# akuhara/RF_INV

Measured on NVIDIA B200. Metric: forward+likelihood evals/sec, higher is better.
Workload: dtype f64

## Files before the change

### rf_inv_b200/build.py

```python
from __future__ import annotations

import os
import shutil
import subprocess
import sys

HERE = os.path.dirname(os.path.abspath(__file__))
CSRC = os.path.join(HERE, "csrc")
SO = os.path.join(HERE, "librfinv_b200.so")
SOURCES = ["capi.cu", "forward.cu", "forward_general.cu", "likelihood.cu", "pt.cu", "comm.cu", "checkpoint.cu", "fp64_peak.cu", "host_io.cu"]
HEADERS = ["rfinv_common.cuh", "rfinv_handle.h", "rfinv_pt.h", os.path.join("..", "..", "include", "rfinv_b200.h")]
NVCC_FLAGS = [
    "-gencode", "arch=compute_100a,code=sm_100a", "-lineinfo", "-O3", "-std=c++17",
    "-Xcompiler", "-fPIC", "-Xcompiler", "-O3", "--expt-relaxed-constexpr", "-Xptxas", "-v",
]


def nvcc_path() -> str:
    for cand in (os.environ.get("NVCC"), shutil.which("nvcc"), "/usr/local/cuda/bin/nvcc"):
        if cand and os.path.exists(cand):
            return cand
    raise RuntimeError("nvcc not found")


def needs_build() -> bool:
    if not os.path.exists(SO):
        return True
    t = os.path.getmtime(SO)
    deps = [os.path.join(CSRC, s) for s in SOURCES + HEADERS] + [os.path.abspath(__file__)]
    return any(os.path.exists(d) and os.path.getmtime(d) > t for d in deps)


def build(force: bool = False, verbose: bool = False) -> str:
    if not force and not needs_build():
        return SO
    objdir = os.path.join(HERE, "build")
    os.makedirs(objdir, exist_ok=True)
    nvcc = nvcc_path()
    objs = []
    procs = []
    env = dict(os.environ)
    host_cxx = "/usr/bin/g++" if os.path.exists("/usr/bin/g++") else "g++"
    for s in SOURCES:
        o = os.path.join(objdir, s.replace(".cu", ".o"))
# ... 23 lines not shown
```

### rf_inv_b200/csrc/capi.cu

```cuda
#include <cstdarg>
#include <cstdio>
#include <cstdlib>
#include <cstring>
#include <cmath>
#include <vector>
#include <algorithm>
#include "rfinv_handle.h"

static thread_local char g_err[1024] = "";

int rfinv_pdl_mode() {
  static const int mode = getenv("RFINV_PDL") ? atoi(getenv("RFINV_PDL")) : 2;
  return mode;
}

int rfinv_arith_switches() {
  auto on = [](const char* name) { return getenv(name) && atoi(getenv(name)) != 0; };
  static const int bits = (on("RFINV_FULL_BAND") ? 1 : 0) | (on("RFINV_QF_DENSE") ? 2 : 0) | (on("RFINV_QF_NOSPLIT") ? 4 : 0);
  return bits;
}

void rfinv_set_error(const char* fmt, ...) {
  va_list ap;
  va_start(ap, fmt);
  vsnprintf(g_err, sizeof(g_err), fmt, ap);
  va_end(ap);
}

namespace {

void build_filter(const rfinv_config& c, std::vector<double>& flt) {
  const int nh = c.nfft / 2 + 1;
  flt.resize((size_t)c.ntrc * nh);
  const double df = 1.0 / (c.delta * c.nfft);
  for (int t = 0; t < c.ntrc; ++t) {
    const double fac_norm = c.nfft * c.a_gus[t] * c.delta / std::sqrt(RFINV_PI);
    for (int i = 0; i < nh; ++i) {
      const double omega = i * 2.0 * RFINV_PI * df;
      const double q = omega / (2.0 * c.a_gus[t]);
      flt[(size_t)t * nh + i] = std::exp(-(q * q)) / fac_norm;
// ... 369 lines not shown
  d.prior_mode = cfg->prior_mode; d.nref = cfg->nref;
  d.ray_common = 1;
  for (int t = 1; t < T; ++t)
    if (cfg->rayps[t] != cfg->rayps[0] || cfg->ipha[t] != cfg->ipha[0]) d.ray_common = 0;
  d.nsmp_pad = ((S + 63) / 64) * 64;
  d.delta = cfg->delta; d.t_start = cfg->t_start; d.sdep = cfg->sdep; d.bdep = cfg->bdep; d.z_ref_min = cfg->z_ref_min; d.dz_ref = cfg->dz_ref;
  d.z_min = cfg->z_min; d.z_max = cfg->z_max; d.h_min = cfg->h_min;
  d.vp_min = cfg->vp_min; d.vp_max = cfg->vp_max; d.vs_min = cfg->vs_min; d.vs_max = cfg->vs_max;
  d.vpvs_min = cfg->vpvs_min; d.vpvs_max = cfg->vpvs_max;
  d.domg = 2.0 * RFINV_PI / (cfg->nfft * cfg->delta);
  for (int t = 0; t < T; ++t) { d.rayp[t] = cfg->rayps[t]; d.ipha[t] = cfg->ipha[t]; }

  std::vector<double> flt;
  build_filter(*cfg, flt);
  band_limits(d, flt);
  std::vector<double2> tw;
  build_twiddles(d.fft_len, tw);
  std::vector<double2> chirp, chirp_b;
  std::vector<double2> twq;
  if (d.fft_general) {
    build_chirp(cfg->nfft, d.fft_len, chirp, chirp_b);
    for (int N = d.fft_len; N > 8; N >>= 3) {
      const int stride = N >> 3, tmul = d.fft_len / N;
      for (int i = 0; i < 7 * stride; ++i) { const int q = i / stride + 1, o = i - (q - 1) * stride; twq.push_back(tw[(size_t)q * o * tmul]); }
    }
  }
  const int Sp = d.nsmp_pad;
  std::vector<double> rpad((size_t)T * Sp * Sp, 0.0);
  for (int t = 0; t < T; ++t)
    for (int i = 0; i < S; ++i)
      for (int j = 0; j < S; ++j)
        rpad[((size_t)t * Sp + i) * Sp + j] =
            0.5 * (h->h_r_inv[((size_t)t * S + i) * S + j] + h->h_r_inv[((size_t)t * S + j) * S + i]);
  std::vector<double> wfac;
  {
    const bool force_dense = (rfinv_arith_switches() & 2) != 0;
    const bool no_split = (rfinv_arith_switches() & 4) != 0;
    const int ntile_dense = Sp / 64;
    std::vector<std::vector<double>> Wt(T);
    std::vector<int> wrows_t(T, 0);
    std::vector<double> a, w, v, a2, w2, v2;
    d.qf_tiles_max = 0;
    int wrows = 64;
    const double rs2 = 0.70710678118654752440;
    for (int t = 0; t < T; ++t) {
      d.qf_rank[t] = 0; d.qf_rank_s[t] = 0; d.qf_split[t] = 0;
      d.qf_tiles[t] = ntile_dense;
      const double* Rm = &rpad[(size_t)t * Sp * Sp];
      auto R = [&](int i, int j) { return Rm[(size_t)i * Sp + j]; };
      int same = -1;
      for (int u = 0; u < t && same < 0; ++u)
        if (std::memcmp(&rpad[(size_t)u * Sp * Sp], Rm, sizeof(double) * (size_t)Sp * Sp) == 0) same = u;
      if (force_dense) {  }
      else if (same >= 0) {
        d.qf_rank[t] = d.qf_rank[same]; d.qf_rank_s[t] = d.qf_rank_s[same]; d.qf_split[t] = d.qf_split[same];
        d.qf_tiles[t] = d.qf_tiles[same]; Wt[t] = Wt[same]; wrows_t[t] = wrows_t[same];
      } else {
        double rmax = 0.0, asym = 0.0;
        for (int i = 0; i < S; ++i)
          for (int j = 0; j < S; ++j) {
            rmax = std::max(rmax, std::fabs(R(i, j)));
            asym = std::max(asym, std::fabs(R(i, j) - R(S - 1 - i, S - 1 - j)));
          }
        const int ha = S / 2, hs = S - ha;
        const bool split = !no_split && rmax > 0.0 && asym <= 1e-10 * rmax && hs <= Sp / 2;
        const double units_dense = 0.5 * ntile_dense * (ntile_dense + 1);
        auto tile_units = [&](int r) { return r / 64 + (r % 64 ? 0.4 : 0.0); };
// ... 62 lines not shown
            for (int e = 0; e < S; ++e) if (w[e] > tol) order.push_back(e);
            std::sort(order.begin(), order.end(), [&](int x, int y) { return w[x] > w[y] || (w[x] == w[y] && x < y); });
            for (int row = 0; row < r; ++row) {
              const int e = order[row];
              const double sc = std::sqrt(w[e]);
              for (int i = 0; i < S; ++i) Wt[t][(size_t)row * Sp + i] = sc * v[(size_t)i * S + e];
            }
          }
        }
      }
      d.qf_tiles_max = std::max(d.qf_tiles_max, d.qf_tiles[t]);
      wrows = std::max(wrows, wrows_t[t]);
    }
    d.qf_wrows = wrows;
    wfac.assign((size_t)T * wrows * Sp, 0.0);
    for (int t = 0; t < T; ++t)
      if (!Wt[t].empty()) std::memcpy(&wfac[(size_t)t * wrows * Sp], Wt[t].data(), sizeof(double) * Wt[t].size());
    {
      int tr = 0;
      for (int t = 0; t < T; ++t) if (d.qf_tiles[t] > d.qf_tiles[tr]) tr = t;
      std::vector<std::pair<double, int>> cost;
      for (int jt = 0; jt < d.qf_tiles_max && jt < RFINV_MAX_QF_TILES; ++jt) {
        double cst;
        if (d.qf_rank[tr] == 0) cst = jt + 1;
        else if (d.qf_split[tr]) {
          const int rs = d.qf_rank_s[tr], ts = (rs + 63) / 64;
          cst = std::min(64, jt < ts ? rs - 64 * jt : (d.qf_rank[tr] - rs) - 64 * (jt - ts));
        } else cst = std::min(64, d.qf_rank[tr] - 64 * jt);
        cost.push_back({-cst, jt});
      }
      std::sort(cost.begin(), cost.end());
      for (size_t q = 0; q < cost.size(); ++q) d.qf_order[q] = cost[q].second;
    }
  }
#define RFINV_TRY(x) do { st = (x); if (st != RFINV_OK) { rfinv_destroy(h); return st; } } while (0)
  RFINV_TRY(upload(flt, &h->d_flt));
  RFINV_TRY(upload(tw, &h->d_tw));
  if (d.fft_general) { RFINV_TRY(upload(chirp, &h->d_chirp)); RFINV_TRY(upload(chirp_b, &h->d_chirp_b)); RFINV_TRY(upload(twq, &h->d_twq)); }
  RFINV_TRY(upload(h->h_obs, &h->d_obs));
  RFINV_TRY(upload(h->h_vp_ref, &h->d_vp_ref));
  RFINV_TRY(upload(h->h_vs_ref, &h->d_vs_ref));
  RFINV_TRY(upload(rpad, &h->d_r_inv));
  RFINV_TRY(upload(wfac, &h->d_w_fac));
#undef RFINV_TRY
  d.flt = h->d_flt; d.tw = h->d_tw; d.chirp = h->d_chirp; d.chirp_b = h->d_chirp_b; d.twq = h->d_twq; d.obs = h->d_obs; d.vp_ref = h->d_vp_ref; d.vs_ref = h->d_vs_ref; d.r_inv = h->d_r_inv; d.w_fac = h->d_w_fac;
  cudaError_t e = cudaStreamCreateWithFlags(&h->stream, cudaStreamNonBlocking);
  if (e != cudaSuccess) { rfinv_set_error("cudaStreamCreate: %s", cudaGetErrorString(e)); rfinv_destroy(h); return RFINV_ERR_CUDA; }
  h->own_stream = true;
  *out = h;
  return RFINV_OK;
}

void rfinv_destroy(rfinv_handle* h) {
  if (!h) return;
  cudaSetDevice(h->device);
  if (h->stream) cudaStreamSynchronize(h->stream);
  h->free_pt();
  rfinv_comm_destroy(h);
  h->free_workspace();
  cudaFree(h->d_flt); cudaFree(h->d_tw); cudaFree(h->d_chirp); cudaFree(h->d_chirp_b); cudaFree(h->d_twq); cudaFree(h->d_obs); cudaFree(h->d_vp_ref); cudaFree(h->d_vs_ref); cudaFree(h->d_r_inv); cudaFree(h->d_w_fac);
  if (h->own_stream && h->stream) cudaStreamDestroy(h->stream);
  if (h->stream_copy) {
    cudaStreamSynchronize(h->stream_copy);
    cudaStreamDestroy(h->stream_copy);
    for (cudaEvent_t e : h->ev_copy) if (e) cudaEventDestroy(e);
  }
  for (int i = 0; i < RFINV_ASYNC_SLOTS; ++i) {
    if (h->async_stream[i]) { cudaStreamSynchronize(h->async_stream[i]); cudaStreamDestroy(h->async_stream[i]); }
    if (h->async_ws[i]) { h->async_ws[i]->release(); delete h->async_ws[i]; }
  }
  for (int i = 0; i < 4; ++i)
    if (h->ev[i]) cudaEventDestroy(h->ev[i]);
  delete h;
}

int32_t rfinv_set_stream(rfinv_handle* h, uint64_t cuda_stream) {
  if (!h) { rfinv_set_error("handle is NULL"); return RFINV_ERR_ARG; }
  if (h->own_stream && h->stream) { cudaStreamSynchronize(h->stream); cudaStreamDestroy(h->stream); }
  h->stream = reinterpret_cast<cudaStream_t>(cuda_stream);
  h->own_stream = false;
  return RFINV_OK;
}

int32_t rfinv_synchronize(rfinv_handle* h) {
  if (!h) { rfinv_set_error("handle is NULL"); return RFINV_ERR_ARG; }
  RFINV_CUDA_CHECK(cudaStreamSynchronize(h->stream));
  return RFINV_OK;
}

int32_t rfinv_last_launch_count(rfinv_handle* h) { return h ? h->launches : 0; }

int32_t rfinv_set_timing(rfinv_handle* h, int32_t enable) {
  if (!h) { rfinv_set_error("handle is NULL"); return RFINV_ERR_ARG; }
// ... 325 lines not shown
```

### rf_inv_b200/csrc/likelihood.cu

```cuda
#include "rfinv_common.cuh"

namespace {

constexpr int TM = 64;
constexpr int TN = 64;
constexpr int TK = 16;
constexpr int LDS_STRIDE = TK + 4;
constexpr int QF_THREADS = 128;
constexpr int QF_CHUNK = 384;

__device__ __forceinline__ void cp_async16(void* smem_dst, const void* gmem_src) {
  const unsigned d = (unsigned)__cvta_generic_to_shared(smem_dst);
  asm volatile("cp.async.cg.shared.global [%0], [%1], 16;\n" ::"r"(d), "l"(gmem_src));
}
__device__ __forceinline__ void cp_async_commit() { asm volatile("cp.async.commit_group;\n" ::); }
template <int N>
__device__ __forceinline__ void cp_async_wait() { asm volatile("cp.async.wait_group %0;\n" ::"n"(N)); }

__device__ __forceinline__ void dmma884(double& c0, double& c1, double a, double b) {
  asm volatile("mma.sync.aligned.m8n8k4.row.col.f64.f64.f64.f64 {%0,%1}, {%2}, {%3}, {%0,%1};\n"
               : "+d"(c0), "+d"(c1) : "d"(a), "d"(b));
}

__global__ void __launch_bounds__(QF_THREADS, 4) quadform_kernel(const DevConfig cfg, int C, const double* __restrict__ misfit,
                                                              double* __restrict__ phi, double* __restrict__ partial,
                                                              int* __restrict__ arrivals, int* __restrict__ work,
                                                              const int* __restrict__ active, int n_active,
                                                              const int* __restrict__ n_active_dev, const double* __restrict__ sig,
                                                              double* __restrict__ logl) {
  __shared__ __align__(16) double sA[2][TM * LDS_STRIDE];
  __shared__ __align__(16) double sB[2][TN * LDS_STRIDE];
  __shared__ int s_rows[TM];
  __shared__ double s_part[2][TM];
  __shared__ int s_next, s_last;
  const int Sp = cfg.nsmp_pad, T = cfg.ntrc;
  const int tid = threadIdx.x, lane = tid & 31, warp = tid >> 5;
  const int wm = warp >> 1, wn = warp & 1;
  const int n_rb_grid = ((active ? n_active : C) + TM - 1) / TM;
  const int ntile = cfg.qf_tiles_max;
  const int n_items = ntile * T * n_rb_grid;
  const int fr = lane >> 2, fk = lane & 3;
  if (tid == 0) s_next = (int)gridDim.x + atomicAdd(work, 1);
  pdl_wait();
  const int n_rows = active ? (n_active_dev ? *n_active_dev : n_active) : C;
  int item = blockIdx.x;
  while (item < n_items) {
    const int nblk = T * n_rb_grid;
    const int chunk = item / (ntile * QF_CHUNK), local = item - chunk * (ntile * QF_CHUNK);
    const int cb = min(QF_CHUNK, nblk - chunk * QF_CHUNK);
    const int jt = cfg.qf_order[local / cb];
    const int blk = chunk * QF_CHUNK + local % cb;
    const int t = blk / n_rb_grid, rb = blk - t * n_rb_grid;
    const int row0 = rb * TM;
    const int rank = cfg.qf_rank[t];
    const int ntile_t = cfg.qf_tiles[t];
    __syncthreads();
    const int next = s_next;
    int next_raw = 0;
    if (tid == 0) next_raw = atomicAdd(work, 1);
    if (row0 < n_rows && jt < ntile_t) {
      if (tid < TM) {
        int r = row0 + tid;
        r = r < n_rows ? r : n_rows - 1;
        s_rows[tid] = active ? active[r] : r;
      }
      __syncthreads();
      const double* __restrict__ Mt = misfit + (size_t)t * C * Sp;
      const double* __restrict__ Rt = rank > 0 ? cfg.w_fac + (size_t)t * cfg.qf_wrows * Sp : cfg.r_inv + (size_t)t * Sp * Sp;
      int jw = 4, koff = 0, nk = (jt + 1) * (TN / TK);
      if (rank > 0) {
        int cols_tile = rank - jt * TN;
        nk = Sp / TK;
        if (cfg.qf_split[t]) {
          const int rs = cfg.qf_rank_s[t], ts = (rs + TN - 1) / TN;
          cols_tile = jt < ts ? rs - jt * TN : (rank - rs) - (jt - ts) * TN;
          koff = jt < ts ? 0 : Sp >> 1;
          nk = (Sp >> 1) / TK;
        }
        const int nfrag = cols_tile >= TN ? 8 : (cols_tile <= 0 ? 0 : (cols_tile + 7) >> 3);
        jw = (nfrag + 1 - wn) >> 1;
      }
      const double* a_src[4];
      int cp_off[4], cp_row[4];
#pragma unroll
      for (int q = 0; q < 4; ++q) {
        const int id = tid + q * QF_THREADS;
        const int row = id >> 3, seg = id & 7;
        cp_row[q] = row;
        cp_off[q] = row * LDS_STRIDE + seg * 2;
        a_src[q] = Mt + (size_t)s_rows[row] * Sp + seg * 2 + koff;
      }
      double acc[4][4][2];
#pragma unroll
      for (int i = 0; i < 4; ++i)
#pragma unroll
        for (int j = 0; j < 4; ++j) acc[i][j][0] = acc[i][j][1] = 0.0;
      const double* b_base = Rt + (size_t)(jt * TN) * Sp + koff;
#pragma unroll
      for (int q = 0; q < 4; ++q) {
        cp_async16(&sA[0][cp_off[q]], a_src[q]);
        cp_async16(&sB[0][cp_off[q]], b_base + (size_t)cp_row[q] * Sp + (cp_off[q] - cp_row[q] * LDS_STRIDE));
      }
      cp_async_commit();
      for (int ks = 0; ks < nk; ++ks) {
        const int cur = ks & 1;
        cp_async_wait<0>();
        __syncthreads();
        if (ks + 1 < nk) {
          const int k0 = (ks + 1) * TK;
#pragma unroll
          for (int q = 0; q < 4; ++q) {
            cp_async16(&sA[cur ^ 1][cp_off[q]], a_src[q] + k0);
            cp_async16(&sB[cur ^ 1][cp_off[q]], b_base + (size_t)cp_row[q] * Sp + k0 + (cp_off[q] - cp_row[q] * LDS_STRIDE));
          }
          cp_async_commit();
        }
        if (rank == 0 && ks == jt * (TN / TK) && jt > 0) {
#pragma unroll
          for (int i = 0; i < 4; ++i)
#pragma unroll
            for (int j = 0; j < 4; ++j) { acc[i][j][0] *= 2.0; acc[i][j][1] *= 2.0; }
        }
        const double* A = &sA[cur][(wm * 32 + fr) * LDS_STRIDE + fk];
        const double* B = &sB[cur][(wn * 8 + fr) * LDS_STRIDE + fk];
#pragma unroll
        for (int kk = 0; kk < TK; kk += 4) {
          double a[4], b[4];
#pragma unroll
          for (int i = 0; i < 4; ++i) a[i] = A[i * 8 * LDS_STRIDE + kk];
#pragma unroll
          for (int j = 0; j < 4; ++j) b[j] = B[j * 16 * LDS_STRIDE + kk];
          if (jw == 4) {
#pragma unroll
            for (int i = 0; i < 4; ++i)
#pragma unroll
              for (int j = 0; j < 4; ++j) dmma884(acc[i][j][0], acc[i][j][1], a[i], b[j]);
          } else {
#pragma unroll
            for (int j = 0; j < 4; ++j)
              if (j < jw) {
#pragma unroll
                for (int i = 0; i < 4; ++i) dmma884(acc[i][j][0], acc[i][j][1], a[i], b[j]);
              }
          }
        }
      }
#pragma unroll
      for (int i = 0; i < 4; ++i) {
        const double* mrow = Mt + (size_t)s_rows[wm * 32 + 8 * i + fr] * Sp + jt * TN + wn * 8 + 2 * fk;
        double v = 0.0;
        if (rank > 0) {
#pragma unroll
          for (int j = 0; j < 4; ++j) { v = fma(acc[i][j][0], acc[i][j][0], v); v = fma(acc[i][j][1], acc[i][j][1], v); }
        } else {
#pragma unroll
          for (int j = 0; j < 4; ++j) {
            const double2 m = *reinterpret_cast<const double2*>(mrow + 16 * j);
            v = fma(acc[i][j][0], m.x, v);
            v = fma(acc[i][j][1], m.y, v);
          }
        }
        v += __shfl_xor_sync(0xffffffffu, v, 1);
        v += __shfl_xor_sync(0xffffffffu, v, 2);
        if (fk == 0) s_part[wn][wm * 32 + 8 * i + fr] = v;
      }
      __syncthreads();
      double* part_t = partial + (size_t)t * C;
      const size_t jstride = (size_t)T * C;
      if (tid < TM && row0 + tid < n_rows) part_t[(size_t)jt * jstride + s_rows[tid]] = s_part[0][tid] + s_part[1][tid];
      __threadfence();
      __syncthreads();
      if (tid == 0) s_last = (atomicAdd(&arrivals[t * n_rb_grid + rb], 1) == ntile_t - 1);
      __syncthreads();
      if (s_last) {
        __threadfence();
        if (tid < TM && row0 + tid < n_rows) {
          const int c = s_rows[tid];
          double v = 0.0;
          for (int j = 0; j < ntile_t; ++j) v += __ldcg(part_t + (size_t)j * jstride + c);
          phi[(size_t)t * C + c] = v;
        }
        if (tid == 0) arrivals[t * n_rb_grid + rb] = 0;
        if (logl) {
          __threadfence();
          __syncthreads();
          if (tid == 0) s_last = (atomicAdd(&arrivals[T * n_rb_grid + rb], 1) == T - 1);
          __syncthreads();
          if (s_last) {
            __threadfence();
            if (tid < TM && row0 + tid < n_rows) {
              const int c = s_rows[tid];
              double ll = 0.0;
              for (int tt = 0; tt < T; ++tt) {
                const double sg = sig[(size_t)tt * C + c];
                const double ph = __ldcg(phi + (size_t)tt * C + c);
                ll = __dsub_rn(__dsub_rn(ll, __ddiv_rn(__dmul_rn(0.5, ph), __dmul_rn(sg, sg))), __dmul_rn((double)cfg.nsmp, log(sg)));
              }
              logl[c] = ll;
            }
            if (tid == 0) arrivals[T * n_rb_grid + rb] = 0;
          }
        }
      }
    } else {
      __syncthreads();
    }
    if (tid == 0) s_next = (int)gridDim.x + next_raw;
    item = next;
  }
  if (tid == 0) {
    __threadfence();
    if (atomicAdd(work + 1, 1) == (int)gridDim.x - 1) { work[0] = 0; work[1] = 0; }
  }
}

__global__ void loglik_kernel(const DevConfig cfg, int C, const double* __restrict__ phi, const double* __restrict__ sig,
                              double* __restrict__ logl) {
  const int c = blockIdx.x * blockDim.x + threadIdx.x;
  if (c >= C) return;
  double ll = 0.0;
  for (int t = 0; t < cfg.ntrc; ++t) {
    const double s = sig[(size_t)t * C + c];
    const double ph = phi[(size_t)t * C + c];
    ll = __dsub_rn(__dsub_rn(ll, __ddiv_rn(__dmul_rn(0.5, ph), __dmul_rn(s, s))), __dmul_rn((double)cfg.nsmp, log(s)));
  }
  logl[c] = ll;
}

}

size_t rfinv_quadform_partial_doubles(const DevConfig& cfg, int C) { return (size_t)(cfg.nsmp_pad / TN + 1) * cfg.ntrc * C; }
size_t rfinv_quadform_counter_ints(const DevConfig& cfg, int C) { return (size_t)((C + TM - 1) / TM) * (cfg.ntrc + 1) + 4; }

int rfinv_launch_quadform(const DevConfig& cfg, int C, const double* misfit, double* phi, double* partial, int* counters,
                          const int* active, int n_active, const int* n_active_dev, cudaStream_t stream, const double* sig,
                          double* logl) {
  const int n_rows = active ? n_active : C;
  if (n_rows == 0) return RFINV_OK;
  const size_t ntile = cfg.qf_tiles_max;
  int* work = counters;
  int* arrivals = counters + 4;
  static int resident_of_device[64] = {0};
  int dev = 0;
  RFINV_CUDA_CHECK(cudaGetDevice(&dev));
  long long resident = (dev >= 0 && dev < 64) ? resident_of_device[dev] : 0;
  if (resident == 0) {
    int per_sm = 0, n_sm = 0;
    RFINV_CUDA_CHECK(cudaDeviceGetAttribute(&n_sm, cudaDevAttrMultiProcessorCount, dev));
    RFINV_CUDA_CHECK(cudaOccupancyMaxActiveBlocksPerMultiprocessor(&per_sm, quadform_kernel, QF_THREADS, 0));
    resident = (long long)n_sm * (per_sm < 1 ? 1 : per_sm);
    if (dev >= 0 && dev < 64) resident_of_device[dev] = (int)resident;
  }
  const long long items = (long long)ntile * cfg.ntrc * ((n_rows + TM - 1) / TM);
  RFINV_CUDA_CHECK(rfinv_launch_pdl(2, quadform_kernel, dim3((unsigned)(items < resident ? items : resident)), dim3(QF_THREADS), 0, stream, cfg, C,
                                    misfit, phi, partial, arrivals, work, active, n_active, n_active_dev, sig, logl));
  return RFINV_OK;
}

int rfinv_launch_loglik(const DevConfig& cfg, int C, const double* phi, const double* sig, double* logl,
                        cudaStream_t stream) {
  if (C == 0) return RFINV_OK;
  loglik_kernel<<<(C + 255) / 256, 256, 0, stream>>>(cfg, C, phi, sig, logl);
  RFINV_CUDA_CHECK(cudaGetLastError());
  return RFINV_OK;
}
```

### rf_inv_b200/csrc/rfinv_common.cuh

```cuda
#pragma once
#include <cuda_runtime.h>
#include <stdint.h>
#include <math.h>
#include <map>
#include <mutex>
#include <utility>
#include "../../include/rfinv_b200.h"

#define RFINV_MAX_TRC 16
#define RFINV_MAX_K 64
#define RFINV_MAX_LAY (RFINV_MAX_K + 2)
#define RFINV_MAX_QF_TILES 64

#define RFINV_PI 3.1415926535897931

struct DevConfig {
  int ntrc, nfft, nh, nsmp;
  int log2n;
  int fft_general, nfft_p2, fft_len;
  int deconv_mode, vp_mode, k_min, k_max, prior_mode, nref, ray_common;
  int nsmp_pad;
  double bdep;
  double delta, t_start, sdep, z_ref_min, dz_ref, z_min, z_max, h_min;
  double vp_min, vp_max, vs_min, vs_max, vpvs_min, vpvs_max;
  double domg;
  double rayp[RFINV_MAX_TRC];
  int ipha[RFINV_MAX_TRC];
  int jbins[RFINV_MAX_TRC];
  int jb_max;
  const double* flt;
  const double2* tw;
  const double2* twq;
  const double2* chirp;
  const double2* chirp_b;
  const double* obs;
  const double* vp_ref;
  const double* vs_ref;
  const double* r_inv;
  const double* w_fac;
  int qf_rank[RFINV_MAX_TRC];
  int qf_split[RFINV_MAX_TRC];
  int qf_rank_s[RFINV_MAX_TRC];
  int qf_tiles[RFINV_MAX_TRC];
  int qf_tiles_max, qf_wrows;
  int qf_order[RFINV_MAX_QF_TILES];
};

struct ModelBatch {
  int C;
  const int* k;
  const double* z;
  const double* dvp;
  const double* dvs;
  const double* sig;
  const int* active;
  int n_active;
  const int* n_active_dev;
  int chain_major = 0;
};

__host__ __device__ __forceinline__ int f_nint(double x) {
  return x >= 0.0 ? (int)floor(x + 0.5) : -(int)floor(-x + 0.5);
}

__device__ __forceinline__ double vp_to_rho(double a1) {
  double a2 = __dmul_rn(a1, a1), a3 = __dmul_rn(a2, a1), a4 = __dmul_rn(a3, a1), a5 = __dmul_rn(a4, a1);
  double p = __dmul_rn((double)1.6612f, a1);
  p = __dsub_rn(p, __dmul_rn((double)0.4721f, a2));
  p = __dadd_rn(p, __dmul_rn((double)0.0671f, a3));
  p = __dsub_rn(p, __dmul_rn((double)0.0043f, a4));
  p = __dadd_rn(p, __dmul_rn((double)0.000106f, a5));
  return p;
}

__device__ __forceinline__ bool layer_velocity(const DevConfig& cfg, double zc, double d_vs, double d_vp, double& alpha,
                                               double& beta) {
  int iz = f_nint(__ddiv_rn(__dsub_rn(zc, cfg.z_ref_min), cfg.dz_ref)) + 1;
  iz = iz < 1 ? 1 : (iz > cfg.nref ? cfg.nref : iz);
// ... 75 lines not shown
```

### rf_inv_b200/csrc/rfinv_handle.h

```cpp
#pragma once
#include <vector>
#include "rfinv_common.cuh"

struct PtState;

struct EvalWorkspace {
  int cap = 0;
  int* d_k = nullptr;
  double *d_z = nullptr, *d_dvp = nullptr, *d_dvs = nullptr, *d_sig = nullptr, *d_stage = nullptr;
  double *d_misfit = nullptr, *d_phi = nullptr, *d_logl = nullptr, *d_rft_full = nullptr, *d_scratch = nullptr;
  uint8_t* d_valid = nullptr;
  double* d_qpart = nullptr;
  int* d_qcnt = nullptr;
  size_t cap_rft_full = 0;
  int grow(const DevConfig& dc, const rfinv_config& cfg, int device, int C);
  void release();
};

constexpr int RFINV_ASYNC_SLOTS = 2;
constexpr int RFINV_UPLOAD_PIECES = 4;

struct rfinv_handle : EvalWorkspace {
  int device = 0;
  cudaStream_t stream = nullptr;
  bool own_stream = false;
  rfinv_config cfg;
  std::vector<double> h_rayps, h_a_gus, h_obs, h_vp_ref, h_vs_ref, h_sig_min, h_sig_max, h_r_inv;
  std::vector<int32_t> h_ipha;
  DevConfig dc;
  double* d_flt = nullptr;
  double2* d_tw = nullptr;
  double2 *d_chirp = nullptr, *d_chirp_b = nullptr, *d_twq = nullptr;
  double* d_obs = nullptr;
  double* d_vp_ref = nullptr;
  double* d_vs_ref = nullptr;
  double* d_r_inv = nullptr;
  double* d_w_fac = nullptr;
  cudaStream_t stream_copy = nullptr;
  cudaEvent_t ev_copy[RFINV_UPLOAD_PIECES + 2] = {};
  EvalWorkspace* async_ws[RFINV_ASYNC_SLOTS] = {};
  cudaStream_t async_stream[RFINV_ASYNC_SLOTS] = {};
  bool async_pending[RFINV_ASYNC_SLOTS] = {};
  int launches = 0;
  bool timing = false;
  cudaEvent_t ev[4] = {nullptr, nullptr, nullptr, nullptr};
  PtState* pt = nullptr;
  void* comm = nullptr;
  int comm_world = 1, comm_rank = 0;

  int ensure_capacity(int C) { if (C > cap) invalidate_pt_graphs(); return grow(dc, cfg, device, C); }
  void invalidate_pt_graphs();
  void free_workspace() { release(); }
  void free_pt();
  int eval_device(int C, const int* k, const double* z, const double* dvp, const double* dvs, const double* sig,
                  double* logl, double* rft_smp, double* rft_full, uint8_t* is_valid, const int* active, int n_active,
                  const ModelBatch* layout = nullptr, EvalWorkspace* w = nullptr, cudaStream_t s = nullptr,
                  bool prep_done = false,
                  cudaEvent_t before_quadform = nullptr);
};

int rfinv_comm_allgather(rfinv_handle* h, const double* send, double* recv, size_t count, cudaStream_t s);
extern "C" int32_t rfinv_comm_destroy(rfinv_handle* h);
int rfinv_comm_peer_setup(rfinv_handle* h);
void rfinv_comm_peer_release(rfinv_handle* h);
int rfinv_pt_fix_assigned_bins(rfinv_handle* h);
int rfinv_pt_reserve_lhist(rfinv_handle* h, int upto);
int rfinv_arith_switches();
```

Baseline: 12.93 million.

## Compute factored quadratic form with int8 tcgen05 MMA via fp64 digit-plane emulation

After: 12.04 million (median of 6 runs). 6.9% lower.

```diff
diff --git a/rf_inv_b200/build.py b/rf_inv_b200/build.py
--- a/rf_inv_b200/build.py
+++ b/rf_inv_b200/build.py
@@ -9,7 +9,7 @@
 CSRC = os.path.join(HERE, "csrc")
 SO = os.path.join(HERE, "librfinv_b200.so")
 SOURCES = ["capi.cu", "forward.cu", "forward_general.cu", "likelihood.cu", "pt.cu", "comm.cu", "checkpoint.cu", "fp64_peak.cu", "host_io.cu"]
-HEADERS = ["rfinv_common.cuh", "rfinv_handle.h", "rfinv_pt.h", os.path.join("..", "..", "include", "rfinv_b200.h")]
+HEADERS = ["rfinv_common.cuh", "qf_int8.cuh", "rfinv_handle.h", "rfinv_pt.h", os.path.join("..", "..", "include", "rfinv_b200.h")]
 NVCC_FLAGS = [
     "-gencode", "arch=compute_100a,code=sm_100a", "-lineinfo", "-O3", "-std=c++17",
     "-Xcompiler", "-fPIC", "-Xcompiler", "-O3", "--expt-relaxed-constexpr", "-Xptxas", "-v",
diff --git a/rf_inv_b200/csrc/capi.cu b/rf_inv_b200/csrc/capi.cu
--- a/rf_inv_b200/csrc/capi.cu
+++ b/rf_inv_b200/csrc/capi.cu
@@ -6,6 +6,7 @@
 #include <vector>
 #include <algorithm>
 #include "rfinv_handle.h"
+#include "qf_int8.cuh"
 
 static thread_local char g_err[1024] = "";
 
@@ -441,7 +442,8 @@
       for (int j = 0; j < S; ++j)
         rpad[((size_t)t * Sp + i) * Sp + j] =
             0.5 * (h->h_r_inv[((size_t)t * S + i) * S + j] + h->h_r_inv[((size_t)t * S + j) * S + i]);
-  std::vector<double> wfac;
+  std::vector<double> wfac, wqs;
+  std::vector<int8_t> wq;
   {
     const bool force_dense = (rfinv_arith_switches() & 2) != 0;
     const bool no_split = (rfinv_arith_switches() & 4) != 0;
@@ -570,6 +572,33 @@
       std::sort(cost.begin(), cost.end());
       for (size_t q = 0; q < cost.size(); ++q) d.qf_order[q] = cost[q].second;
     }
+    const int nsl = Sp / QI_SW;
+    const size_t slab_bytes = (size_t)QI_PLANES * QI_TN * QI_SW, tile_bytes = nsl * slab_bytes;
+    wq.assign((size_t)T * d.qf_tiles_max * tile_bytes, 0);
+    wqs.assign((size_t)T * wrows, 0.0);
+    for (int t = 0; t < T; ++t) {
+      if (d.qf_rank[t] == 0) continue;
+      const int K = d.qf_split[t] ? Sp / 2 : Sp, ts = d.qf_split[t] ? (d.qf_rank_s[t] + 63) / 64 : d.qf_tiles[t];
+      if (K > QI_KMAX || K % QI_SW) { rfinv_set_error("quadratic form: K = %d outside the exact int8 range", K); rfinv_destroy(h); return RFINV_ERR_ARG; }
+      for (int jt = 0; jt < d.qf_tiles[t]; ++jt) {
+        const int koff = jt < ts ? 0 : Sp / 2;
+        int8_t* tile = &wq[((size_t)t * d.qf_tiles_max + jt) * tile_bytes];
+        for (int n = 0; n < QI_TN; ++n) {
+          const double* col = &wfac[((size_t)t * wrows + 64 * jt + n) * Sp + koff];
+          uint32_t mx = 0;
+          for (int k = 0; k < K; ++k) { uint64_t b; std::memcpy(&b, &col[k], 8); mx = std::max(mx, (uint32_t)(b >> 32) & 0x7fffffffu); }
+          const int E = qi_exp(mx);
+          const double sc = qi_scale_in(E);
+          wqs[(size_t)t * wrows + 64 * jt + n] = qi_scale_out(E);
+          for (int k = 0; k < K; ++k) {
+            uint32_t lo, hi;
+            qi_digits(col[k] * sc, lo, hi);
+            int8_t* slab = tile + (size_t)(k / QI_SW) * slab_bytes + qi_sw_offset(n, (k % QI_SW) >> 4) + (k & 15);
+            for (int p = 0; p < QI_PLANES; ++p) slab[(size_t)p * QI_TN * QI_SW] = qi_plane_byte(lo, hi, p);
+          }
+        }
+      }
+    }
   }
 #define RFINV_TRY(x) do { st = (x); if (st != RFINV_OK) { rfinv_destroy(h); return st; } } while (0)
   RFINV_TRY(upload(flt, &h->d_flt));
@@ -579,9 +608,10 @@
   RFINV_TRY(upload(h->h_vp_ref, &h->d_vp_ref));
   RFINV_TRY(upload(h->h_vs_ref, &h->d_vs_ref));
   RFINV_TRY(upload(rpad, &h->d_r_inv));
-  RFINV_TRY(upload(wfac, &h->d_w_fac));
+  RFINV_TRY(upload(wq, &h->d_w_q));
+  RFINV_TRY(upload(wqs, &h->d_w_qscale));
 #undef RFINV_TRY
-  d.flt = h->d_flt; d.tw = h->d_tw; d.chirp = h->d_chirp; d.chirp_b = h->d_chirp_b; d.twq = h->d_twq; d.obs = h->d_obs; d.vp_ref = h->d_vp_ref; d.vs_ref = h->d_vs_ref; d.r_inv = h->d_r_inv; d.w_fac = h->d_w_fac;
+  d.flt = h->d_flt; d.tw = h->d_tw; d.chirp = h->d_chirp; d.chirp_b = h->d_chirp_b; d.twq = h->d_twq; d.obs = h->d_obs; d.vp_ref = h->d_vp_ref; d.vs_ref = h->d_vs_ref; d.r_inv = h->d_r_inv; d.w_q = h->d_w_q; d.w_qscale = h->d_w_qscale;
   cudaError_t e = cudaStreamCreateWithFlags(&h->stream, cudaStreamNonBlocking);
   if (e != cudaSuccess) { rfinv_set_error("cudaStreamCreate: %s", cudaGetErrorString(e)); rfinv_destroy(h); return RFINV_ERR_CUDA; }
   h->own_stream = true;
@@ -596,7 +626,7 @@
   h->free_pt();
   rfinv_comm_destroy(h);
   h->free_workspace();
-  cudaFree(h->d_flt); cudaFree(h->d_tw); cudaFree(h->d_chirp); cudaFree(h->d_chirp_b); cudaFree(h->d_twq); cudaFree(h->d_obs); cudaFree(h->d_vp_ref); cudaFree(h->d_vs_ref); cudaFree(h->d_r_inv); cudaFree(h->d_w_fac);
+  cudaFree(h->d_flt); cudaFree(h->d_tw); cudaFree(h->d_chirp); cudaFree(h->d_chirp_b); cudaFree(h->d_twq); cudaFree(h->d_obs); cudaFree(h->d_vp_ref); cudaFree(h->d_vs_ref); cudaFree(h->d_r_inv); cudaFree(h->d_w_q); cudaFree(h->d_w_qscale);
   if (h->own_stream && h->stream) cudaStreamDestroy(h->stream);
   if (h->stream_copy) {
     cudaStreamSynchronize(h->stream_copy);
diff --git a/rf_inv_b200/csrc/likelihood.cu b/rf_inv_b200/csrc/likelihood.cu
--- a/rf_inv_b200/csrc/likelihood.cu
+++ b/rf_inv_b200/csrc/likelihood.cu
@@ -1,4 +1,5 @@
 #include "rfinv_common.cuh"
+#include "qf_int8.cuh"
 
 namespace {
 
@@ -52,8 +53,7 @@
     const int blk = chunk * QF_CHUNK + local % cb;
     const int t = blk / n_rb_grid, rb = blk - t * n_rb_grid;
     const int row0 = rb * TM;
-    const int rank = cfg.qf_rank[t];
-    const int ntile_t = cfg.qf_tiles[t];
+    const int ntile_t = cfg.qf_rank[t] == 0 ? cfg.qf_tiles[t] : 0;
     __syncthreads();
     const int next = s_next;
     int next_raw = 0;
@@ -66,20 +66,8 @@
       }
       __syncthreads();
       const double* __restrict__ Mt = misfit + (size_t)t * C * Sp;
-      const double* __restrict__ Rt = rank > 0 ? cfg.w_fac + (size_t)t * cfg.qf_wrows * Sp : cfg.r_inv + (size_t)t * Sp * Sp;
-      int jw = 4, koff = 0, nk = (jt + 1) * (TN / TK);
-      if (rank > 0) {
-        int cols_tile = rank - jt * TN;
-        nk = Sp / TK;
-        if (cfg.qf_split[t]) {
-          const int rs = cfg.qf_rank_s[t], ts = (rs + TN - 1) / TN;
-          cols_tile = jt < ts ? rs - jt * TN : (rank - rs) - (jt - ts) * TN;
-          koff = jt < ts ? 0 : Sp >> 1;
-          nk = (Sp >> 1) / TK;
-        }
-        const int nfrag = cols_tile >= TN ? 8 : (cols_tile <= 0 ? 0 : (cols_tile + 7) >> 3);
-        jw = (nfrag + 1 - wn) >> 1;
-      }
+      const double* __restrict__ Rt = cfg.r_inv + (size_t)t * Sp * Sp;
+      const int nk = (jt + 1) * (TN / TK);
       const double* a_src[4];
       int cp_off[4], cp_row[4];
 #pragma unroll
@@ -88,14 +76,14 @@
         const int row = id >> 3, seg = id & 7;
         cp_row[q] = row;
         cp_off[q] = row * LDS_STRIDE + seg * 2;
-        a_src[q] = Mt + (size_t)s_rows[row] * Sp + seg * 2 + koff;
+        a_src[q] = Mt + (size_t)s_rows[row] * Sp + seg * 2;
       }
       double acc[4][4][2];
 #pragma unroll
       for (int i = 0; i < 4; ++i)
 #pragma unroll
         for (int j = 0; j < 4; ++j) acc[i][j][0] = acc[i][j][1] = 0.0;
-      const double* b_base = Rt + (size_t)(jt * TN) * Sp + koff;
+      const double* b_base = Rt + (size_t)(jt * TN) * Sp;
 #pragma unroll
       for (int q = 0; q < 4; ++q) {
         cp_async16(&sA[0][cp_off[q]], a_src[q]);
@@ -115,7 +103,7 @@
           }
           cp_async_commit();
         }
-        if (rank == 0 && ks == jt * (TN / TK) && jt > 0) {
+        if (ks == jt * (TN / TK) && jt > 0) {
 #pragma unroll
           for (int i = 0; i < 4; ++i)
 #pragma unroll
@@ -130,35 +118,21 @@
           for (int i = 0; i < 4; ++i) a[i] = A[i * 8 * LDS_STRIDE + kk];
 #pragma unroll
           for (int j = 0; j < 4; ++j) b[j] = B[j * 16 * LDS_STRIDE + kk];
-          if (jw == 4) {
-#pragma unroll
-            for (int i = 0; i < 4; ++i)
-#pragma unroll
-              for (int j = 0; j < 4; ++j) dmma884(acc[i][j][0], acc[i][j][1], a[i], b[j]);
-          } else {
-#pragma unroll
-            for (int j = 0; j < 4; ++j)
-              if (j < jw) {
-#pragma unroll
-                for (int i = 0; i < 4; ++i) dmma884(acc[i][j][0], acc[i][j][1], a[i], b[j]);
-              }
-          }
+#pragma unroll
+          for (int i = 0; i < 4; ++i)
+#pragma unroll
+            for (int j = 0; j < 4; ++j) dmma884(acc[i][j][0], acc[i][j][1], a[i], b[j]);
         }
       }
 #pragma unroll
       for (int i = 0; i < 4; ++i) {
         const double* mrow = Mt + (size_t)s_rows[wm * 32 + 8 * i + fr] * Sp + jt * TN + wn * 8 + 2 * fk;
         double v = 0.0;
-        if (rank > 0) {
-#pragma unroll
-          for (int j = 0; j < 4; ++j) { v = fma(acc[i][j][0], acc[i][j][0], v); v = fma(acc[i][j][1], acc[i][j][1], v); }
-        } else {
-#pragma unroll
-          for (int j = 0; j < 4; ++j) {
-            const double2 m = *reinterpret_cast<const double2*>(mrow + 16 * j);
-            v = fma(acc[i][j][0], m.x, v);
-            v = fma(acc[i][j][1], m.y, v);
-          }
+#pragma unroll
+        for (int j = 0; j < 4; ++j) {
+          const double2 m = *reinterpret_cast<const double2*>(mrow + 16 * j);
+          v = fma(acc[i][j][0], m.x, v);
+          v = fma(acc[i][j][1], m.y, v);
         }
         v += __shfl_xor_sync(0xffffffffu, v, 1);
         v += __shfl_xor_sync(0xffffffffu, v, 2);
@@ -214,6 +188,238 @@
   }
 }
 
+constexpr int QI_THREADS = 256;
+constexpr int QI_STAGES = 4;
+constexpr int QI_A_BYTES = QI_PLANES * QI_TM * QI_SW;
+constexpr int QI_B_BYTES = QI_PLANES * QI_TN * QI_SW;
+constexpr int QI_SMEM = QI_STAGES * (QI_A_BYTES + QI_B_BYTES) + 1024;
+constexpr int QI_CHUNK = 192;
+constexpr int QI_TMEM_COLS = 512;
+
+__global__ void __launch_bounds__(QI_THREADS, 1) quadform_int8_kernel(const DevConfig cfg, int C, const double* __restrict__ misfit,
+                                                                   double* __restrict__ phi, double* __restrict__ partial,
+                                                                   int* __restrict__ arrivals, int* __restrict__ work,
+                                                                   const int* __restrict__ active, int n_active,
+                                                                   const int* __restrict__ n_active_dev, const double* __restrict__ sig,
+                                                                   double* __restrict__ logl, int n_trc_logl) {
+  extern __shared__ unsigned char qi_smem_raw[];
+  unsigned char* const sA = (unsigned char*)(((uintptr_t)qi_smem_raw + 1023) & ~(uintptr_t)1023);
+  unsigned char* const sB = sA + QI_STAGES * QI_A_BYTES;
+  __shared__ uint64_t s_bar[QI_STAGES];
+  __shared__ uint32_t s_tmem;
+  __shared__ int s_rows[QI_TM], s_exp[QI_TM];
+  __shared__ double s_part[2][QI_TM];
+  __shared__ int s_next, s_last;
+  const int Sp = cfg.nsmp_pad, T = cfg.ntrc;
+  const int tid = threadIdx.x, lane = tid & 31, warp = tid >> 5;
+  const int n_rb_grid = ((active ? n_active : C) + QI_TM - 1) / QI_TM;
+  const int ntile = cfg.qf_tiles_max;
+  const int n_items = ntile * T * n_rb_grid;
+  if (tid == 0) {
+    s_next = (int)gridDim.x + atomicAdd(work, 1);
+    for (int b = 0; b < QI_STAGES; ++b) qi_bar_init(&s_bar[b], 1);
+    asm volatile("fence.mbarrier_init.release.cluster;" ::: "memory");
+  }
+  if (warp == 0) qi_tmem_alloc(&s_tmem, QI_TMEM_COLS);
+  qi_fence_before();
+  __syncthreads();
+  qi_fence_after();
+  const uint32_t tmem = s_tmem;
+  pdl_wait();
+  const int n_rows = active ? (n_active_dev ? *n_active_dev : n_active) : C;
+  const int prow = tid >> 1, pc = tid & 1;
+  uint32_t g = 0;
+  int item = blockIdx.x;
+  while (item < n_items) {
+    const int nblk = T * n_rb_grid;
+    const int chunk = item / (ntile * QI_CHUNK), local = item - chunk * (ntile * QI_CHUNK);
+    const int cb = min(QI_CHUNK, nblk - chunk * QI_CHUNK);
+    const int jt = cfg.qf_order[local / cb];
+    const int blk = chunk * QI_CHUNK + local % cb;
+    const int t = blk / n_rb_grid, rb = blk - t * n_rb_grid;
+    const int row0 = rb * QI_TM;
+    const int rank = cfg.qf_rank[t];
+    const int ntile_t = rank > 0 ? cfg.qf_tiles[t] : 0;
+    __syncthreads();
+    const int next = s_next;
+    int next_raw = 0;
+    if (tid == 0) next_raw = atomicAdd(work, 1);
+    if (row0 < n_rows && jt < ntile_t) {
+      if (tid < QI_TM) {
+        int r = row0 + tid;
+        r = r < n_rows ? r : n_rows - 1;
+        s_rows[tid] = active ? active[r] : r;
+      }
+      int cols = rank - jt * QI_TN, koff = 0, K = Sp;
+      if (cfg.qf_split[t]) {
+        const int rs = cfg.qf_rank_s[t], ts = (rs + QI_TN - 1) / QI_TN;
+        cols = jt < ts ? rs - jt * QI_TN : (rank - rs) - (jt - ts) * QI_TN;
+        koff = jt < ts ? 0 : Sp >> 1;
+        K = Sp >> 1;
+      }
+      cols = min(cols, QI_TN);
+      const int n_mma = (cols + 15) & ~15;
+      const int nslab = K / QI_SW;
+      const double* __restrict__ Mt = misfit + (size_t)t * C * Sp + koff;
+      __syncthreads();
+      for (int r = warp; r < QI_TM; r += QI_THREADS / 32) {
+        const double* src = Mt + (size_t)s_rows[r] * Sp;
+        uint32_t mx = 0;
+#pragma unroll 4
+        for (int k = 2 * lane; k < K; k += 64) {
+          const double2 x = *reinterpret_cast<const double2*>(src + k);
+          mx = max(mx, max((uint32_t)__double2hiint(x.x) & 0x7fffffffu, (uint32_t)__double2hiint(x.y) & 0x7fffffffu));
+        }
+        mx = __reduce_max_sync(0xffffffffu, mx);
+        if (lane == 0) s_exp[r] = qi_exp(mx);
+      }
+      __syncthreads();
+      const double* psrc = Mt + (size_t)s_rows[prow] * Sp + pc * 16;
+      const double pscale = qi_scale_in(s_exp[prow]);
+      const int poff = qi_sw_offset(prow, pc);
+      const int8_t* wsrc = cfg.w_q + ((size_t)t * ntile + jt) * (size_t)(Sp / QI_SW) * QI_B_BYTES;
+      const uint32_t idesc = qi_idesc(n_mma);
+      auto stage_free = [&](uint32_t gg) {
+        if (gg >= QI_STAGES) qi_bar_wait(&s_bar[gg % QI_STAGES], ((gg / QI_STAGES) - 1) & 1);
+      };
+      auto copy_b = [&](int s, uint32_t gg) {
+        unsigned char* dst = sB + (gg % QI_STAGES) * QI_B_BYTES;
+        const int8_t* src = wsrc + (size_t)s * QI_B_BYTES;
+        for (int i = tid; i < QI_B_BYTES / 16; i += QI_THREADS)
+          if (((i >> 1) & (QI_TN - 1)) < n_mma) cp_async16(dst + 16 * i, src + 16 * i);
+        cp_async_commit();
+      };
+      double2 xn[8];
+      auto load_a = [&](int s) {
+#pragma unroll
+        for (int q = 0; q < 8; ++q) xn[q] = reinterpret_cast<const double2*>(psrc + s * QI_SW)[q];
+      };
+      stage_free(g);
+      copy_b(0, g);
+      load_a(0);
+      for (int s = 0; s < nslab; ++s, ++g) {
+        double x[16];
+#pragma unroll
+        for (int q = 0; q < 8; ++q) { x[2 * q] = xn[q].x; x[2 * q + 1] = xn[q].y; }
+        if (s + 1 < nslab) { stage_free(g + 1); copy_b(s + 1, g + 1); load_a(s + 1); }
+        unsigned char* dA = sA + (g % QI_STAGES) * QI_A_BYTES + poff;
+        uint32_t lo[16], hi[16];
+#pragma unroll
+        for (int e = 0; e < 16; ++e) qi_digits(x[e] * pscale, lo[e], hi[e]);
+        uint4 pl[QI_PLANES];
+#pragma unroll
+        for (int q = 0; q < 4; ++q) {
+          const uint32_t* L = lo + 4 * q;
+          const uint32_t* H = hi + 4 * q;
+          const uint32_t l01 = __byte_perm(L[0], L[1], 0x5140), l23 = __byte_perm(L[2], L[3], 0x5140);
+          const uint32_t h01 = __byte_perm(L[0], L[1], 0x7362), h23 = __byte_perm(L[2], L[3], 0x7362);
+          const uint32_t m01 = __byte_perm(H[0], H[1], 0x5140), m23 = __byte_perm(H[2], H[3], 0x5140);
+          const uint32_t t01 = __byte_perm(H[0], H[1], 0x7362), t23 = __byte_perm(H[2], H[3], 0x7362);
+          const uint32_t w[QI_PLANES] = {__byte_perm(t01, t23, 0x5410),
+                                         __byte_perm(m01, m23, 0x7632),
+                                         __byte_perm(m01, m23, 0x5410),
+                                         __byte_perm(h01, h23, 0x7632),
+                                         __byte_perm(h01, h23, 0x5410),
+                                         __byte_perm(l01, l23, 0x7632),
+                                         __byte_perm(l01, l23, 0x5410)};
+#pragma unroll
+          for (int p = 0; p < QI_PLANES; ++p) (&pl[p].x)[q] = w[p];
+        }
+#pragma unroll
+        for (int p = 0; p < QI_PLANES; ++p) *reinterpret_cast<uint4*>(dA + p * QI_TM * QI_SW) = pl[p];
+        if (s + 1 < nslab) cp_async_wait<1>(); else cp_async_wait<0>();
+        qi_fence_async_smem();
+        __syncthreads();
+        if (tid == 0) {
+          qi_fence_after();
+          const uint32_t a0 = qi_smem_u32(sA + (g % QI_STAGES) * QI_A_BYTES), b0 = qi_smem_u32(sB + (g % QI_STAGES) * QI_B_BYTES);
+#pragma unroll
+          for (int i = 0; i < QI_PLANES; ++i)
+#pragma unroll
+            for (int j = 0; i + j < QI_PLANES; ++j)
+              qi_mma(tmem + (uint32_t)((i + j) * QI_TN), qi_smem_desc(a0 + i * QI_TM * QI_SW), qi_smem_desc(b0 + j * QI_TN * QI_SW),
+                     idesc, s > 0 || i > 0);
+          qi_commit(&s_bar[g % QI_STAGES]);
+        }
+      }
+      qi_bar_wait(&s_bar[(g - 1) % QI_STAGES], ((g - 1) / QI_STAGES) & 1);
+      qi_fence_after();
+      {
+        const int lb = 32 * (warp & 3), ch = warp >> 2, row = lb + lane;
+        const double* wsc = cfg.w_qscale + (size_t)t * cfg.qf_wrows + jt * QI_TN;
+        double v = 0.0;
+        for (int c0 = 32 * ch; c0 < 32 * ch + 32 && c0 < cols; c0 += 8) {
+          int d[QI_DIAGS][8];
+#pragma unroll
+          for (int dd = 0; dd < QI_DIAGS; ++dd) qi_tmem_ld8(tmem + ((uint32_t)lb << 16) + (uint32_t)(dd * QI_TN + c0), d[dd]);
+          qi_tmem_wait_ld();
+#pragma unroll
+          for (int q = 0; q < 8; ++q) {
+            double h = (double)d[QI_DIAGS - 1][q];
+#pragma unroll
+            for (int dd = QI_DIAGS - 2; dd >= 0; --dd) h = fma(h, 0x1p-8, (double)d[dd][q]);
+            const double z = h * wsc[c0 + q];
+            v = fma(z, z, v);
+          }
+        }
+        const int E = s_exp[row];
+        const double so = qi_scale_out(E);
+        s_part[ch][row] = E == 2047 ? __longlong_as_double(0x7ff8000000000000ll) : v * so * so;
+      }
+      qi_fence_before();
+      __syncthreads();
+      double* part_t = partial + (size_t)t * C;
+      const size_t jstride = (size_t)T * C;
+      if (tid < QI_TM && row0 + tid < n_rows) part_t[(size_t)jt * jstride + s_rows[tid]] = s_part[0][tid] + s_part[1][tid];
+      __threadfence();
+      __syncthreads();
+      if (tid == 0) s_last = (atomicAdd(&arrivals[t * n_rb_grid + rb], 1) == ntile_t - 1);
+      __syncthreads();
+      if (s_last) {
+        __threadfence();
+        if (tid < QI_TM && row0 + tid < n_rows) {
+          const int c = s_rows[tid];
+          double v = 0.0;
+          for (int j = 0; j < ntile_t; ++j) v += __ldcg(part_t + (size_t)j * jstride + c);
+          phi[(size_t)t * C + c] = v;
+        }
+        if (tid == 0) arrivals[t * n_rb_grid + rb] = 0;
+        if (logl) {
+          __threadfence();
+          __syncthreads();
+          if (tid == 0) s_last = (atomicAdd(&arrivals[T * n_rb_grid + rb], 1) == n_trc_logl - 1);
+          __syncthreads();
+          if (s_last) {
+            __threadfence();
+            if (tid < QI_TM && row0 + tid < n_rows) {
+              const int c = s_rows[tid];
+              double ll = 0.0;
+              for (int tt = 0; tt < T; ++tt) {
+                const double sg = sig[(size_t)tt * C + c];
+                const double ph = __ldcg(phi + (size_t)tt * C + c);
+                ll = __dsub_rn(__dsub_rn(ll, __ddiv_rn(__dmul_rn(0.5, ph), __dmul_rn(sg, sg))), __dmul_rn((double)cfg.nsmp, log(sg)));
+              }
+              logl[c] = ll;
+            }
+            if (tid == 0) arrivals[T * n_rb_grid + rb] = 0;
+          }
+        }
+      }
+    } else {
+      __syncthreads();
+    }
+    if (tid == 0) s_next = (int)gridDim.x + next_raw;
+    item = next;
+  }
+  qi_fence_before();
+  __syncthreads();
+  if (warp == 0) qi_tmem_free(tmem, QI_TMEM_COLS);
+  if (tid == 0) {
+    __threadfence();
+    if (atomicAdd(work + 1, 1) == (int)gridDim.x - 1) { work[0] = 0; work[1] = 0; }
+  }
+}
+
 __global__ void loglik_kernel(const DevConfig cfg, int C, const double* __restrict__ phi, const double* __restrict__ sig,
                               double* __restrict__ logl) {
   const int c = blockIdx.x * blockDim.x + threadIdx.x;
@@ -230,7 +436,25 @@
 }
 
 size_t rfinv_quadform_partial_doubles(const DevConfig& cfg, int C) { return (size_t)(cfg.nsmp_pad / TN + 1) * cfg.ntrc * C; }
-size_t rfinv_quadform_counter_ints(const DevConfig& cfg, int C) { return (size_t)((C + TM - 1) / TM) * (cfg.ntrc + 1) + 4; }
+static size_t dense_counter_ints(const DevConfig& cfg, int C) { return (size_t)((C + TM - 1) / TM) * (cfg.ntrc + 1) + 4; }
+size_t rfinv_quadform_counter_ints(const DevConfig& cfg, int C) {
+  return dense_counter_ints(cfg, C) + (size_t)((C + QI_TM - 1) / QI_TM) * (cfg.ntrc + 1) + 4;
+}
+
+template <typename K>
+static int resident_ctas(K kernel, int threads, size_t smem, int (&cache)[64], long long* resident) {
+  int dev = 0;
+  RFINV_CUDA_CHECK(cudaGetDevice(&dev));
+  *resident = (dev >= 0 && dev < 64) ? cache[dev] : 0;
+  if (*resident == 0) {
+    int per_sm = 0, n_sm = 0;
+    RFINV_CUDA_CHECK(cudaDeviceGetAttribute(&n_sm, cudaDevAttrMultiProcessorCount, dev));
+    RFINV_CUDA_CHECK(cudaOccupancyMaxActiveBlocksPerMultiprocessor(&per_sm, kernel, threads, smem));
+    *resident = (long long)n_sm * (per_sm < 1 ? 1 : per_sm);
+    if (dev >= 0 && dev < 64) cache[dev] = (int)*resident;
+  }
+  return RFINV_OK;
+}
 
 int rfinv_launch_quadform(const DevConfig& cfg, int C, const double* misfit, double* phi, double* partial, int* counters,
                           const int* active, int n_active, const int* n_active_dev, cudaStream_t stream, const double* sig,
@@ -238,22 +462,29 @@
   const int n_rows = active ? n_active : C;
   if (n_rows == 0) return RFINV_OK;
   const size_t ntile = cfg.qf_tiles_max;
-  int* work = counters;
-  int* arrivals = counters + 4;
-  static int resident_of_device[64] = {0};
-  int dev = 0;
-  RFINV_CUDA_CHECK(cudaGetDevice(&dev));
-  long long resident = (dev >= 0 && dev < 64) ? resident_of_device[dev] : 0;
-  if (resident == 0) {
-    int per_sm = 0, n_sm = 0;
-    RFINV_CUDA_CHECK(cudaDeviceGetAttribute(&n_sm, cudaDevAttrMultiProcessorCount, dev));
-    RFINV_CUDA_CHECK(cudaOccupancyMaxActiveBlocksPerMultiprocessor(&per_sm, quadform_kernel, QF_THREADS, 0));
-    resident = (long long)n_sm * (per_sm < 1 ? 1 : per_sm);
-    if (dev >= 0 && dev < 64) resident_of_device[dev] = (int)resident;
-  }
-  const long long items = (long long)ntile * cfg.ntrc * ((n_rows + TM - 1) / TM);
-  RFINV_CUDA_CHECK(rfinv_launch_pdl(2, quadform_kernel, dim3((unsigned)(items < resident ? items : resident)), dim3(QF_THREADS), 0, stream, cfg, C,
-                                    misfit, phi, partial, arrivals, work, active, n_active, n_active_dev, sig, logl));
+  int n_factor = 0;
+  for (int t = 0; t < cfg.ntrc; ++t) n_factor += cfg.qf_rank[t] > 0;
+  const int n_dense = cfg.ntrc - n_factor;
+  if (n_dense > 0) {
+    static int resident_of_device[64] = {0};
+    long long resident = 0;
+    if (resident_ctas(quadform_kernel, QF_THREADS, 0, resident_of_device, &resident) != RFINV_OK) return RFINV_ERR_CUDA;
+    const long long items = (long long)ntile * cfg.ntrc * ((n_rows + TM - 1) / TM);
+    RFINV_CUDA_CHECK(rfinv_launch_pdl(2, quadform_kernel, dim3((unsigned)(items < resident ? items : resident)), dim3(QF_THREADS), 0, stream,
+                                      cfg, C, misfit, phi, partial, counters + 4, counters, active, n_active, n_active_dev, sig,
+                                      n_factor > 0 ? nullptr : logl));
+  }
+  if (n_factor > 0) {
+    int* cnt = counters + dense_counter_ints(cfg, C);
+    RFINV_CUDA_CHECK(rfinv_raise_smem_limit((const void*)quadform_int8_kernel, QI_SMEM));
+    static int resident_of_device[64] = {0};
+    long long resident = 0;
+    if (resident_ctas(quadform_int8_kernel, QI_THREADS, QI_SMEM, resident_of_device, &resident) != RFINV_OK) return RFINV_ERR_CUDA;
+    const long long items = (long long)ntile * cfg.ntrc * ((n_rows + QI_TM - 1) / QI_TM);
+    RFINV_CUDA_CHECK(rfinv_launch_pdl(2, quadform_int8_kernel, dim3((unsigned)(items < resident ? items : resident)), dim3(QI_THREADS),
+                                      QI_SMEM, stream, cfg, C, misfit, phi, partial, cnt + 4, cnt, active, n_active, n_active_dev, sig,
+                                      logl, n_factor));
+  }
   return RFINV_OK;
 }
 
diff --git a/rf_inv_b200/csrc/qf_int8.cuh b/rf_inv_b200/csrc/qf_int8.cuh
--- /dev/null
+++ b/rf_inv_b200/csrc/qf_int8.cuh
@@ -0,0 +1,81 @@
+#pragma once
+#include <stdint.h>
+#include <string.h>
+
+#define QI_PLANES 7
+#define QI_DIAGS 7
+#define QI_SW 32
+#define QI_MMA_K 32
+#define QI_TM 128
+#define QI_TN 64
+#define QI_KMAX 18723
+
+__host__ __device__ __forceinline__ int qi_exp(uint32_t hi_abs_max) {
+  const int E = (int)(hi_abs_max >> 20);
+  return E < 64 ? 64 : E;
+}
+__host__ __device__ __forceinline__ double qi_bits_to_double(uint64_t b) {
+#ifdef __CUDA_ARCH__
+  return __longlong_as_double((long long)b);
+#else
+  double d; memcpy(&d, &b, 8); return d;
+#endif
+}
+__host__ __device__ __forceinline__ double qi_scale_in(int E) { return qi_bits_to_double((uint64_t)(2099 - E) << 52); }
+__host__ __device__ __forceinline__ double qi_scale_out(int E) { return qi_bits_to_double((uint64_t)(E - 5) << 52); }
+
+__host__ __device__ __forceinline__ void qi_digits(double xs, uint32_t& lo, uint32_t& hi) {
+#ifdef __CUDA_ARCH__
+  const long long v = __double2ll_rn(xs);
+#else
+  const long long v = llrint(xs);
+#endif
+  const unsigned long long u = (unsigned long long)v + 0x808080808080ull;
+  lo = (uint32_t)u ^ 0x80808080u;
+  hi = (uint32_t)(u >> 32) ^ 0x8080u;
+}
+__host__ __device__ __forceinline__ int8_t qi_plane_byte(uint32_t lo, uint32_t hi, int p) {
+  return (int8_t)(p >= 3 ? (lo >> (8 * (6 - p))) & 0xff : (hi >> (8 * (2 - p))) & 0xff);
+}
+
+__host__ __device__ __forceinline__ int qi_sw_offset(int row, int chunk) { return row * QI_SW + ((chunk ^ ((row >> 2) & 1)) << 4); }
+
+#ifdef __CUDACC__
+__device__ __forceinline__ uint64_t qi_smem_desc(uint32_t saddr) {
+  return (uint64_t)((saddr & 0x3FFFF) >> 4) | ((uint64_t)1 << 16) | ((uint64_t)((8 * QI_SW) >> 4) << 32) | ((uint64_t)1 << 46) |
+         ((uint64_t)6 << 61);
+}
+__host__ __device__ __forceinline__ uint32_t qi_idesc(int n) {
+  return (2u << 4) | (1u << 7) | (1u << 10) | ((uint32_t)(n >> 3) << 17) | ((uint32_t)(QI_TM >> 4) << 24);
+}
+__device__ __forceinline__ uint32_t qi_smem_u32(const void* p) { return (uint32_t)__cvta_generic_to_shared(p); }
+__device__ __forceinline__ void qi_mma(uint32_t tmem_d, uint64_t adesc, uint64_t bdesc, uint32_t idesc, uint32_t accum) {
+  asm volatile("{\n.reg .pred p;\nsetp.ne.b32 p, %4, 0;\ntcgen05.mma.cta_group::1.kind::i8 [%0], %1, %2, %3, p;\n}\n"
+               :: "r"(tmem_d), "l"(adesc), "l"(bdesc), "r"(idesc), "r"(accum));
+}
+__device__ __forceinline__ void qi_commit(uint64_t* bar) {
+  asm volatile("tcgen05.commit.cta_group::1.mbarrier::arrive::one.shared::cluster.b64 [%0];" :: "r"(qi_smem_u32(bar)) : "memory");
+}
+__device__ __forceinline__ void qi_bar_init(uint64_t* bar, int count) {
+  asm volatile("mbarrier.init.shared::cta.b64 [%0], %1;" :: "r"(qi_smem_u32(bar)), "r"(count) : "memory");
+}
+__device__ __forceinline__ void qi_bar_wait(uint64_t* bar, uint32_t parity) {
+  asm volatile("{\n.reg .pred P1;\nWAIT_%=:\nmbarrier.try_wait.parity.shared::cta.b64 P1, [%0], %1;\n@!P1 bra WAIT_%=;\n}\n"
+               :: "r"(qi_smem_u32(bar)), "r"(parity) : "memory");
+}
+__device__ __forceinline__ void qi_fence_async_smem() { asm volatile("fence.proxy.async.shared::cta;" ::: "memory"); }
+__device__ __forceinline__ void qi_fence_before() { asm volatile("tcgen05.fence::before_thread_sync;" ::: "memory"); }
+__device__ __forceinline__ void qi_fence_after() { asm volatile("tcgen05.fence::after_thread_sync;" ::: "memory"); }
+__device__ __forceinline__ void qi_tmem_alloc(uint32_t* dst, int ncols) {
+  asm volatile("tcgen05.alloc.cta_group::1.sync.aligned.shared::cta.b32 [%0], %1;\n"
+               "tcgen05.relinquish_alloc_permit.cta_group::1.sync.aligned;\n" :: "r"(qi_smem_u32(dst)), "r"(ncols) : "memory");
+}
+__device__ __forceinline__ void qi_tmem_free(uint32_t taddr, int ncols) {
+  asm volatile("tcgen05.dealloc.cta_group::1.sync.aligned.b32 %0, %1;" :: "r"(taddr), "r"(ncols) : "memory");
+}
+__device__ __forceinline__ void qi_tmem_ld8(uint32_t taddr, int* v) {
+  asm volatile("tcgen05.ld.sync.aligned.32x32b.x8.b32 {%0,%1,%2,%3,%4,%5,%6,%7}, [%8];"
+               : "=r"(v[0]), "=r"(v[1]), "=r"(v[2]), "=r"(v[3]), "=r"(v[4]), "=r"(v[5]), "=r"(v[6]), "=r"(v[7]) : "r"(taddr));
+}
+__device__ __forceinline__ void qi_tmem_wait_ld() { asm volatile("tcgen05.wait::ld.sync.aligned;" ::: "memory"); }
+#endif
diff --git a/rf_inv_b200/csrc/rfinv_common.cuh b/rf_inv_b200/csrc/rfinv_common.cuh
--- a/rf_inv_b200/csrc/rfinv_common.cuh
+++ b/rf_inv_b200/csrc/rfinv_common.cuh
@@ -37,13 +37,14 @@
   const double* vp_ref;
   const double* vs_ref;
   const double* r_inv;
-  const double* w_fac;
   int qf_rank[RFINV_MAX_TRC];
   int qf_split[RFINV_MAX_TRC];
   int qf_rank_s[RFINV_MAX_TRC];
   int qf_tiles[RFINV_MAX_TRC];
   int qf_tiles_max, qf_wrows;
   int qf_order[RFINV_MAX_QF_TILES];
+  const int8_t* w_q;
+  const double* w_qscale;
 };
 
 struct ModelBatch {
diff --git a/rf_inv_b200/csrc/rfinv_handle.h b/rf_inv_b200/csrc/rfinv_handle.h
--- a/rf_inv_b200/csrc/rfinv_handle.h
+++ b/rf_inv_b200/csrc/rfinv_handle.h
@@ -35,7 +35,8 @@
   double* d_vp_ref = nullptr;
   double* d_vs_ref = nullptr;
   double* d_r_inv = nullptr;
-  double* d_w_fac = nullptr;
+  int8_t* d_w_q = nullptr;
+  double* d_w_qscale = nullptr;
   cudaStream_t stream_copy = nullptr;
   cudaEvent_t ev_copy[RFINV_UPLOAD_PIECES + 2] = {};
   EvalWorkspace* async_ws[RFINV_ASYNC_SLOTS] = {};
```
